# max-andr/joint-cnn-mrf

Measured on AMD Instinct MI355X. Metric: images/sec (720x480, K=9 joints) part-detector+spatial-model fwd, higher is better.
Workload: dtype f32(fp16x2 spectra, fft); 1 GPU; configs[1]: batch=64/GPU synthetic 480x720x3, part detector + spatial model forward + argmax, fp32; batch_per_gpu=64, global_batch=64, micro_batch=64, use_sm=True, collective=all_gather coords int32 [B,2,9]

## Files before the change

include/jcm.h:

```cpp
#ifndef JCM_H
#define JCM_H

#include <stddef.h>
#include <stdint.h>

#ifdef __cplusplus
extern "C" {
#endif

typedef struct jcm_ctx* jcm_handle;

#define JCM_OK 0
#define JCM_ERR_ARG 1
#define JCM_ERR_STATE 2
#define JCM_ERR_HIP 3

#define JCM_PRECISION_F32 0
#define JCM_PRECISION_BF16 1

int jcm_create(int device, void* stream, jcm_handle* out);
int jcm_destroy(jcm_handle h);
const char* jcm_last_error(void);
int jcm_abi_version(void);

// ... 54 lines not shown
                    int32_t* disp, int64_t* sad);

int jcm_seq_tracks_viterbi(jcm_handle h, const float* hm, int S, int T, int HH, int WW, int M, const double* taps, int R, double rho, int D,
                           int32_t* path, double* maxes, int32_t* breaks, float* value);
int jcm_seq_tracks_filter(jcm_handle h, const float* hm, int S, int T, int HH, int WW, int M, const double* taps, int R, double rho, int D,
                          const double* state_in, float* filtered, int32_t* coords, double* norm, int32_t* reset, double* state_out, float* value);

int jcm_torso_infer(jcm_handle h, const float* prob, int B, int HH, int WW, int K, const int32_t* cells_in,
                    float* energy, int32_t* cell, float* torso);

int jcm_forward(jcm_handle h, const float* x, const float* torso, int B, int H, int W, int use_sm,
                float* pd_prob, float* sm_prob, int32_t* pd_coords, int32_t* sm_coords);

int jcm_eval_forward(jcm_handle h, const float* x, const float* y, int B, int H, int W, int use_sm,
                     float* pd_prob, float* sm_prob, int32_t* pd_coords, int32_t* sm_coords, float* losses);

int jcm_pd_forward_u8(jcm_handle h, const uint8_t* x, int B, int H, int W, float* logits_out);
int jcm_forward_u8(jcm_handle h, const uint8_t* x, const float* torso, int B, int H, int W, int use_sm,
                   float* pd_prob, float* sm_prob, int32_t* pd_coords, int32_t* sm_coords);
int jcm_eval_forward_u8(jcm_handle h, const uint8_t* x, const float* y, int B, int H, int W, int use_sm,
                        float* pd_prob, float* sm_prob, int32_t* pd_coords, int32_t* sm_coords, float* losses);

int jcm_window_resize(jcm_handle h, const float* src, int nsrc, int H, int W, int C, const int32_t* windows, int NW,
                      int OH, int OW, float* out);
int jcm_group_mean(jcm_handle h, const float* in, int n, int G, int64_t M, float* out);

int jcm_fit_images(jcm_handle h, const uint8_t* src, int64_t src_bytes, const int64_t* desc, int B, int C,
                   int OH, int OW, int pad, int out_f32, void* out, int32_t* geom);

int jcm_fit_windows(jcm_handle h, const uint8_t* src, int64_t src_bytes, const int64_t* desc, int NW, int C,
// ... 94 lines not shown
```

joint-cnn-mrf_amd/_lib.py:

```python
import ctypes
import os

_HERE = os.path.dirname(os.path.abspath(__file__))
LIB_PATH = os.environ.get('JCM_LIB') or os.path.join(_HERE, 'libjcm.so')

JCM_PRECISION_F32 = 0
JCM_PRECISION_BF16 = 1
JCM_OPT_ADAM = 0
JCM_OPT_MOMENTUM = 1
JCM_HIST_BUCKETS = 1551
SYNTH_REC_INTS, SYNTH_PRIM_INTS = 20, 16
HM_FLIP_PERM = (3, 4, 5, 0, 1, 2, 7, 6, 8, 9)

_c_float_p = ctypes.c_void_p
_c_i32_p = ctypes.c_void_p
_handle = ctypes.c_void_p
GRAD_READY_FN = ctypes.CFUNCTYPE(None, ctypes.c_void_p, ctypes.c_int64, ctypes.c_int64)

SIGNATURES = {
    'jcm_create': (ctypes.c_int, [ctypes.c_int, ctypes.c_void_p, ctypes.POINTER(_handle)]),
    'jcm_destroy': (ctypes.c_int, [_handle]),
    'jcm_last_error': (ctypes.c_char_p, []),
    'jcm_abi_version': (ctypes.c_int, []),
    'jcm_set_option': (ctypes.c_int, [_handle, ctypes.c_char_p, ctypes.c_int64]),
# ... 38 lines not shown
                                      ctypes.c_void_p]),
    'jcm_seq_smooth_lag': (ctypes.c_int, [_handle, _c_float_p, ctypes.c_int, ctypes.c_int, ctypes.c_int, ctypes.c_int, ctypes.c_int, ctypes.c_int,
                                          ctypes.POINTER(ctypes.c_double), ctypes.c_int, ctypes.c_double, ctypes.c_int, ctypes.c_int, ctypes.c_void_p,
                                          ctypes.c_void_p, _c_i32_p, _c_float_p, _c_i32_p, _c_float_p, ctypes.c_void_p, _c_i32_p]),
    'jcm_seq_tracks_viterbi': (ctypes.c_int, [_handle, _c_float_p, ctypes.c_int, ctypes.c_int, ctypes.c_int, ctypes.c_int, ctypes.c_int,
                                              ctypes.POINTER(ctypes.c_double), ctypes.c_int, ctypes.c_double, ctypes.c_int, _c_i32_p, ctypes.c_void_p, _c_i32_p,
                                              _c_float_p]),
    'jcm_seq_tracks_filter': (ctypes.c_int, [_handle, _c_float_p, ctypes.c_int, ctypes.c_int, ctypes.c_int, ctypes.c_int, ctypes.c_int,
                                             ctypes.POINTER(ctypes.c_double), ctypes.c_int, ctypes.c_double, ctypes.c_int, ctypes.c_void_p, _c_float_p, _c_i32_p,
                                             ctypes.c_void_p, _c_i32_p, ctypes.c_void_p, _c_float_p]),
    'jcm_frame_shift': (ctypes.c_int, [_handle, ctypes.c_void_p, ctypes.c_int, ctypes.c_int, ctypes.c_int, ctypes.c_int, ctypes.c_int, ctypes.c_int, ctypes.c_int,
                                       ctypes.c_int, ctypes.c_void_p, _c_i32_p, ctypes.c_void_p]),
    'jcm_torso_infer': (ctypes.c_int, [_handle, _c_float_p, ctypes.c_int, ctypes.c_int, ctypes.c_int, ctypes.c_int, _c_i32_p, _c_float_p, _c_i32_p, _c_float_p]),
    'jcm_forward': (ctypes.c_int, [_handle, _c_float_p, _c_float_p, ctypes.c_int, ctypes.c_int, ctypes.c_int, ctypes.c_int,
                                   _c_float_p, _c_float_p, _c_i32_p, _c_i32_p]),
    'jcm_eval_forward': (ctypes.c_int, [_handle, _c_float_p, _c_float_p, ctypes.c_int, ctypes.c_int, ctypes.c_int, ctypes.c_int,
                                        _c_float_p, _c_float_p, _c_i32_p, _c_i32_p, _c_float_p]),
    'jcm_pd_forward_u8': (ctypes.c_int, [_handle, ctypes.c_void_p, ctypes.c_int, ctypes.c_int, ctypes.c_int, _c_float_p]),
    'jcm_forward_u8': (ctypes.c_int, [_handle, ctypes.c_void_p, _c_float_p, ctypes.c_int, ctypes.c_int, ctypes.c_int, ctypes.c_int,
                                      _c_float_p, _c_float_p, _c_i32_p, _c_i32_p]),
    'jcm_eval_forward_u8': (ctypes.c_int, [_handle, ctypes.c_void_p, _c_float_p, ctypes.c_int, ctypes.c_int, ctypes.c_int, ctypes.c_int,
                                           _c_float_p, _c_float_p, _c_i32_p, _c_i32_p, _c_float_p]),
    'jcm_window_resize': (ctypes.c_int, [_handle, _c_float_p, ctypes.c_int, ctypes.c_int, ctypes.c_int, ctypes.c_int,
                                         ctypes.POINTER(ctypes.c_int32), ctypes.c_int, ctypes.c_int, ctypes.c_int, _c_float_p]),
    'jcm_fit_images': (ctypes.c_int, [_handle, ctypes.c_void_p, ctypes.c_int64, ctypes.POINTER(ctypes.c_int64), ctypes.c_int, ctypes.c_int, ctypes.c_int,
                                      ctypes.c_int, ctypes.c_int, ctypes.c_int, ctypes.c_void_p, ctypes.POINTER(ctypes.c_int32)]),
    'jcm_fit_windows': (ctypes.c_int, [_handle, ctypes.c_void_p, ctypes.c_int64, ctypes.POINTER(ctypes.c_int64), ctypes.c_int, ctypes.c_int, ctypes.c_int,
                                       ctypes.c_int, ctypes.c_int, ctypes.c_int, ctypes.c_void_p, ctypes.POINTER(ctypes.c_int32)]),
    'jcm_render_poses': (ctypes.c_int, [_handle, ctypes.c_void_p, ctypes.c_int64, ctypes.POINTER(ctypes.c_int64), ctypes.c_int, ctypes.c_void_p,
                                        ctypes.POINTER(ctypes.c_int32), ctypes.c_int, _c_float_p, ctypes.c_int, ctypes.c_int, ctypes.c_int, ctypes.c_int,
# ... 113 lines not shown
```

joint-cnn-mrf_amd/csrc/ctx.h:

```cpp
#pragma once
#include "../../include/jcm.h"

#include <map>
#include <mutex>
#include <string>
#include <vector>

#include "kernels.h"

namespace jcm {

struct CallOrder;

int fail(int code, const std::string& msg);

#define HIP_TRY(expr)                                                                                   \
  do {                                                                                                  \
    hipError_t e_ = (expr);                                                                             \
    if (e_ != hipSuccess)                                                                               \
      return ::jcm::fail(JCM_ERR_HIP, std::string(#expr) + ": " + hipGetErrorString(e_));               \
  } while (0)
#define JCM_TRY(expr)          \
  do {                         \
    int r_ = (expr);           \
// ... 51 lines not shown
  int device = 0;
  hipStream_t stream = nullptr;
  int precision = JCM_PRECISION_F32;
  int K = 9;
  bool finalized = false;
  int f32_conv = 0;
  int split_min_wgs = 128;
  int sm_algo = 3;
  int conv9_fft = 1;
  int fft_tiles = 1;
  int fft_logits_rows = 1;
  int fft_fuse = 7;
  int fft_single = 1;
  int fft_t16 = 1;
  int fft_rows_mfma = 1;
  int fft_reg = 1;
  int fft_cache_gb = 64;
  int fft_win = 1;
  int bf16_hpool = 1;
  int torso_algo = 1;
  int sm_chunk = 32;
  int micro_batch = 0;
  int call_order = 1;
  int debug_skip = 0;
  std::map<std::string, jcm::Tensor> params;
  std::map<std::string, jcm::ConvLayer> convs;
  std::vector<void*> owned;
  size_t param_bytes = 0;
  bool has_sm = false;
  float* sp_energy = nullptr;
// ... 150 lines not shown
template <class F>
int with_arena(jcm_ctx* c, F&& body) {
  return with_arena(c, body, body);
}

bool conv1_pool_fused(const jcm_ctx* c, const ConvLayer* L1, int H, int W);
bool conv1_split_route(const jcm_ctx* c, const ConvLayer* L1);
int conv1_pool_stage(jcm_ctx* c, const std::string& scope, const ConvLayer* L1, const void* xin, bool xin_u8, int B, int xh, int xw, int xsub, void* dst, void** p1);
struct Pool2Layout {
  int pl23;
  int hp;
};
Pool2Layout pool2_layout(jcm_ctx* c, const ConvLayer* L2, const ConvLayer* L3, int B, int h2, int w2);
hipError_t pool2_launch(jcm_ctx* c, const Pool2Layout& l, const void* c2, void* p2, int B, int h2, int w2, int C);
int pd_forward_impl(jcm_ctx* c, const void* x, bool x_u8, int B, int H, int W, float* logits);
int sm_forward_impl(jcm_ctx* c, const float* hm, int Ca, const float* extra, int B, float* logits, int extra_ld = 0);

}
```

joint-cnn-mrf_amd/csrc/jcm_api.hip:

```cpp
#include <algorithm>
#include <cmath>
#include <cstdlib>
#include <cstdio>
#include <cstring>

#include <mutex>
#include <vector>

#include "ctx.h"
#include "options.h"

using namespace jcm;

namespace {
thread_local std::string g_err;
}

namespace jcm {

const char* const kJointNames[10] = {"lsho", "lelb", "lwri", "rsho", "relb", "rwri", "lhip", "rhip", "nose", "torso"};

int fail(int code, const std::string& msg) {
  g_err = msg;
  return code;
// ... 594 lines not shown
  CallOrder order(h);
  HIP_TRY(softmax_argmax(logits, prob, coords, B, HH * WW, WW, K, h->stream));
  return JCM_OK;
}

int jcm_argmax_coords(jcm_handle h, const float* hm, int B, int HH, int WW, int K, int32_t* coords) {
  JCM_TRY(check(h, false));
  if (!hm || !coords || B < 1 || HH < 1 || WW < 1 || K < 1) return fail(JCM_ERR_ARG, "bad argmax arguments");
  DeviceGuard g(h->device);
  CallOrder order(h);
  HIP_TRY(argmax_coords(hm, coords, B, HH * WW, WW, K, h->stream));
  return JCM_OK;
}

static int forward_impl(jcm_handle h, const void* x, bool x_u8, const float* torso, const float* y, int B, int H, int W, int use_sm,
                        float* pd_prob, float* sm_prob, int32_t* pd_coords, int32_t* sm_coords, float* losses) {
  JCM_TRY(check(h, true));
  if (!x || B < 1 || H < 8 || W < 8) return fail(JCM_ERR_ARG, "bad forward arguments");
  const int tld = y ? h->K + 1 : 1;
  if (y) torso = y + h->K;
  if (use_sm && !torso) return fail(JCM_ERR_ARG, "use_sm needs the torso heat map (y_in[...,K:], main.py:528)");
  if (use_sm && (cdiv2(cdiv2(cdiv2(H))) != kHmH || cdiv2(cdiv2(cdiv2(W))) != kHmW))
    return fail(JCM_ERR_ARG, "the spatial model is defined for 60x90 heat maps (480x720 images) only");
  DeviceGuard g(h->device);
  CallOrder order(h);
  jcm_ctx* c = h;
  const int K = c->K;
  if (use_sm && K + 1 != kC) return fail(JCM_ERR_ARG, "use_sm requires n_joints == 9 (10-channel spatial model)");
  const int hh = cdiv2(cdiv2(cdiv2(H))), ww = cdiv2(cdiv2(cdiv2(W)));
  const int mb_opt = c->micro_batch > 0 ? c->micro_batch : (c->precision == JCM_PRECISION_BF16 ? 256 : 64);
  const int mb = B < mb_opt ? B : mb_opt;
  auto body = [&](int b0, int nb) {
    const size_t n = (size_t)nb * hh * ww * K;
    const size_t o = (size_t)b0 * hh * ww * K;
    float* logits = arena_alloc<float>(c, n);
    float* prob = pd_prob ? pd_prob + o : arena_alloc<float>(c, n);
    const size_t mark = c->arena_off;
    const void* xb = static_cast<const char*>(x) + (size_t)b0 * H * W * 3 * (x_u8 ? 1 : sizeof(float));
    JCM_TRY(pd_forward_impl(c, xb, x_u8, nb, H, W, logits));
    c->arena_off = mark;
    if (!c->dry) HIP_TRY(softmax_argmax(logits, prob, pd_coords ? pd_coords + (size_t)b0 * 2 * K : nullptr, nb, hh * ww, ww, K, c->stream));
    float* ce = losses ? arena_alloc<float>(c, 2 * (size_t)nb * K) : nullptr;
    const float* yb = y ? y + (size_t)b0 * hh * ww * (K + 1) : nullptr;
    if (losses && !c->dry) HIP_TRY(softmax_ce(logits, yb, nb, hh * ww, K, K + 1, 0.f, ce, nullptr, 0, 0, c->stream));
    if (use_sm) {
      float* sml = arena_alloc<float>(c, n);
      float* smp = sm_prob ? sm_prob + o : nullptr;
      hipEvent_t s0 = nullptr, s1 = nullptr;
      if (!c->dry) JCM_TRY(prof_begin(c, &s0, &s1));
      const int rs = sm_forward_impl(c, prob, K, torso + (size_t)b0 * hh * ww * tld, nb, sml, tld);
      if (!c->dry) prof_end(c, "sm", s0, s1, rs == JCM_OK);
      JCM_TRY(rs);
      if (!c->dry && (smp || sm_coords))
        HIP_TRY(softmax_argmax(sml, smp, sm_coords ? sm_coords + (size_t)b0 * 2 * K : nullptr, nb, hh * ww, ww, K, c->stream));
      if (losses && !c->dry) HIP_TRY(softmax_ce(sml, yb, nb, hh * ww, K, K + 1, 0.f, ce + (size_t)nb * K, nullptr, 0, 0, c->stream));
    } else if (losses && !c->dry) {
      HIP_TRY(hipMemcpyAsync(ce + (size_t)nb * K, ce, (size_t)nb * K * sizeof(float), hipMemcpyDeviceToDevice, c->stream));
    }
    if (losses && !c->dry) HIP_TRY(loss_means_accumulate(ce, nb * K, 1.0f / (float)(B * K), losses, b0 == 0, c->stream));
    return (int)JCM_OK;
  };
  return with_arena(c, [&] { return body(0, mb); }, [&] {
    for (int b0 = 0; b0 < B; b0 += mb) {
      c->arena_off = 0;
      JCM_TRY(body(b0, B - b0 < mb ? B - b0 : mb));
    }
    return (int)JCM_OK;
  });
}

int jcm_forward(jcm_handle h, const float* x, const float* torso, int B, int H, int W, int use_sm,
                float* pd_prob, float* sm_prob, int32_t* pd_coords, int32_t* sm_coords) {
  return forward_impl(h, x, false, torso, nullptr, B, H, W, use_sm, pd_prob, sm_prob, pd_coords, sm_coords, nullptr);
}
int jcm_forward_u8(jcm_handle h, const uint8_t* x, const float* torso, int B, int H, int W, int use_sm,
                   float* pd_prob, float* sm_prob, int32_t* pd_coords, int32_t* sm_coords) {
  return forward_impl(h, x, true, torso, nullptr, B, H, W, use_sm, pd_prob, sm_prob, pd_coords, sm_coords, nullptr);
}

int jcm_eval_forward(jcm_handle h, const float* x, const float* y, int B, int H, int W, int use_sm,
                     float* pd_prob, float* sm_prob, int32_t* pd_coords, int32_t* sm_coords, float* losses) {
  if (!y || !losses) return fail(JCM_ERR_ARG, "eval_forward needs the target heat maps y [B,60,90,K+1] and a 2-float loss buffer");
  return forward_impl(h, x, false, nullptr, y, B, H, W, use_sm, pd_prob, sm_prob, pd_coords, sm_coords, losses);
}
int jcm_eval_forward_u8(jcm_handle h, const uint8_t* x, const float* y, int B, int H, int W, int use_sm,
                        float* pd_prob, float* sm_prob, int32_t* pd_coords, int32_t* sm_coords, float* losses) {
  if (!y || !losses) return fail(JCM_ERR_ARG, "eval_forward needs the target heat maps y [B,60,90,K+1] and a 2-float loss buffer");
  return forward_impl(h, x, true, nullptr, y, B, H, W, use_sm, pd_prob, sm_prob, pd_coords, sm_coords, losses);
// ... 390 lines not shown
```

joint-cnn-mrf_amd/csrc/kernels.h:

```cpp
#pragma once
#include <hip/hip_runtime.h>
#include <stdint.h>

#include <atomic>

namespace jcm {

struct LdsAttr {
  std::atomic<uint64_t> done{0};
  hipError_t ensure(const void* fn, int bytes) {
    int dev = 0;
    hipError_t e = hipGetDevice(&dev);
    if (e != hipSuccess) return e;
    const uint64_t bit = 1ull << (dev & 63);
    if (done.load(std::memory_order_acquire) & bit) return hipSuccess;
    e = hipFuncSetAttribute(fn, hipFuncAttributeMaxDynamicSharedMemorySize, bytes);
    if (e == hipSuccess) done.fetch_or(bit, std::memory_order_release);
    return e;
  }
};

struct ConvArgs {
  const void* x;
  const void* wp;
// ... 259 lines not shown

hipError_t sm_softplus5(const float* in, float* out, int64_t n, hipStream_t st);
hipError_t sm_softplus5_multi(const float* const* in, float* out, int P, int64_t n, hipStream_t st);
hipError_t sm_likelihood(const float* hm, int Ca, const float* extra, const float* bn_scale, const float* bn_shift, float* lik,
                         int B, int C, hipStream_t st, int extra_ld = 0);
hipError_t sm_pair_conv(const float* priors, const float* maps, const int* cond, float* cpre,
                        int B, int P, int C, hipStream_t st);
hipError_t sm_finish(const float* lik, const float* cpre, const float* spbias, float* logits,
                     int B, int K, int C, hipStream_t st);
hipError_t sm_resize_only(const float* cpre, float* out, int B, hipStream_t st);

hipError_t sm_pad_frame(const float* hm, int Ca, const float* extra, const float* sc, const float* sh, float* frame, int B, int C,
                        hipStream_t st, int extra_ld = 0);
hipError_t sm_spec_mul(const float2* lhat, const float2* phat, const int* cond, float2* spec, int B, int C, int P, hipStream_t st);
hipError_t sm_resize_frame(const float* cfull, float* out, int B, hipStream_t st);
hipError_t sm_fused_forward(const float* hm, int Ca, const float* extra, int extra_ld, const float* sc, const float* sh, const float2* phat_t,
                            const int* cond, const float* spbias, float2* lhat_t, float* logits, int B, int K, int C, hipStream_t st,
                            float* tsave, void* scratch, unsigned epoch);
size_t sm_fused_scratch_bytes();
hipError_t sm_fused_spectra(const float* hm, int Ca, const float* extra, int extra_ld, const float* sc, const float* sh, float2* lhat_t, int B, int C,
                            hipStream_t st);
hipError_t sm_lds_fwd_frames(const float* frames, float2* spec_t, int n, hipStream_t st);
hipError_t sm_lds_fwd_dframes(const float* G, const float* T, float2* dhat_t, int nb, int K, int P, hipStream_t st);
hipError_t sm_lds_inv_frames(const float2* spec_t, float* frames, int n, int r0, int nrows, float scale, hipStream_t st);

hipError_t window_resize(const float* src, int H, int W, int C, const int* windows_dev, int NW, float2* mm_scratch,
                         int OH, int OW, float* out, hipStream_t st);
hipError_t group_mean(const float* in, float* out, int n, int G, size_t M, hipStream_t st);

size_t augment_scratch_doubles(int B);
hipError_t augment_train(const float* x, const float* y, const float* params, int B, int H, int W, int hh, int hw, double* scratch,
                         float* x_out, float* y_out, hipStream_t st);

// ... 79 lines not shown
```

joint-cnn-mrf_amd/csrc/options.h:

```cpp
#pragma once
#include <climits>

#include "ctx.h"

namespace jcm {

struct Option {
  enum Kind { BOOL, RANGE, EITHER };
  const char* name;
  int jcm_ctx::*field;
  Kind kind;
  int64_t lo, hi;
  bool before_finalize;
  const char* env;
  int (*on_change)(jcm_ctx*, int64_t);
};

int option_profile(jcm_ctx* c, int64_t value);
int option_fft_single(jcm_ctx* c, int64_t value);

inline constexpr Option kOptions[] = {
    {"precision",       &jcm_ctx::precision,       Option::RANGE,  0,  1,       true,  nullptr,               nullptr},
    {"n_joints",        &jcm_ctx::K,               Option::RANGE,  1,  9,       true,  nullptr,               nullptr},
    {"f32_conv",        &jcm_ctx::f32_conv,        Option::EITHER, 0,  2,       true,  nullptr,               nullptr},
    {"split_min_wgs",   &jcm_ctx::split_min_wgs,   Option::RANGE,  0,  INT_MAX, false, nullptr,               nullptr},
    {"profile",         &jcm_ctx::profile,         Option::BOOL,   0,  1,       false, nullptr,               option_profile},
    {"conv9_fft",       &jcm_ctx::conv9_fft,       Option::BOOL,   0,  1,       false, nullptr,               nullptr},
    {"call_order",      &jcm_ctx::call_order,      Option::BOOL,   0,  1,       false, nullptr,               nullptr},
    {"fft_single",      &jcm_ctx::fft_single,      Option::BOOL,   0,  1,       false, nullptr,               option_fft_single},
    {"fft_t16",         &jcm_ctx::fft_t16,         Option::BOOL,   0,  1,       false, nullptr,               nullptr},
    {"fft_rows_mfma",   &jcm_ctx::fft_rows_mfma,   Option::BOOL,   0,  1,       false, nullptr,               nullptr},
    {"fft_windows",     &jcm_ctx::fft_win,         Option::BOOL,   0,  1,       false, nullptr,               nullptr},
    {"fft_fuse",        &jcm_ctx::fft_fuse,        Option::RANGE,  0,  7,       false, nullptr,               nullptr},
    {"fft_tiles",       &jcm_ctx::fft_tiles,       Option::BOOL,   0,  1,       false, "JCM_FFT_TILES",       nullptr},
    {"fft_logits_rows", &jcm_ctx::fft_logits_rows, Option::BOOL,   0,  1,       false, "JCM_FFT_LOGITS_ROWS", nullptr},
    {"fft_reg",         &jcm_ctx::fft_reg,         Option::BOOL,   0,  1,       false, "JCM_FFT_REG",         nullptr},
    {"fft_cache_gb",    &jcm_ctx::fft_cache_gb,    Option::RANGE,  0,  1 << 20, false, "JCM_FFT_CACHE_GB",    nullptr},
    {"bf16_hpool",      &jcm_ctx::bf16_hpool,      Option::BOOL,   0,  1,       false, nullptr,               nullptr},
    {"sm_algo",         &jcm_ctx::sm_algo,         Option::EITHER, 1,  3,       false, nullptr,               nullptr},
    {"torso_algo",      &jcm_ctx::torso_algo,      Option::EITHER, 1,  1,       false, nullptr,               nullptr},
    {"sm_chunk",        &jcm_ctx::sm_chunk,        Option::RANGE,  1,  INT_MAX, false, nullptr,               nullptr},
    {"micro_batch",     &jcm_ctx::micro_batch,     Option::RANGE,  0,  INT_MAX, false, nullptr,               nullptr},
    {"debug_skip",      &jcm_ctx::debug_skip,      Option::RANGE,  0,  127,     false, nullptr,               nullptr},
};

}
```

joint-cnn-mrf_amd/csrc/pd_tower.hip:

```cpp
#include <string>
#include <utility>

#include "ctx.h"

namespace jcm {

bool conv1_pool_fused(const jcm_ctx* c, const ConvLayer* L1, int H, int W) {
  return (c->precision == JCM_PRECISION_BF16 ? L1->wq1_bf16 != nullptr : L1->wq1_f32 != nullptr) && H % 4 == 0 && W % 4 == 0;
}
bool conv1_split_route(const jcm_ctx* c, const ConvLayer* L1) { return c->conv9_fft && c->f32_conv == 0 && L1->wq1_split; }

int conv1_pool_stage(jcm_ctx* c, const std::string& scope, const ConvLayer* L1, const void* xin, bool xin_u8, int B, int xh, int xw, int xsub, void* dst, void** p1) {
  const bool bf = c->precision == JCM_PRECISION_BF16;
  const size_t es = bf ? 2 : 4;
  auto act = [&](size_t elems) { return static_cast<void*>(arena_alloc<char>(c, elems * es)); };
  const int h1 = cdiv2(xh / xsub), w1 = cdiv2(xw / xsub);
  const int h2 = cdiv2(h1), w2 = cdiv2(w1);
  if (conv1_pool_fused(c, L1, xh / xsub, xw / xsub)) {
    *p1 = dst ? dst : act((size_t)B * h2 * w2 * L1->cout);
    if (c->dry) return JCM_OK;
    if (bf) {
      HIP_TRY(conv1_mfma_pool(xin, L1->wq1_bf16, L1->bias, L1->scale, L1->shift, *p1, B, xh, xw, xsub, c->stream, xin_u8));
    } else {
      HIP_TRY(conv1_split_route(c, L1) ? conv1_mfma_pool_split(xin, L1->wq1_split, L1->bias, L1->scale, L1->shift, static_cast<float*>(*p1), B, xh, xw, xsub, c->stream, xin_u8)
// ... 204 lines not shown
  }
  const int sk = c->debug_skip;
  void* t56 = (sk & 96) ? nullptr : offer_handover(c, L5, conv_of(c, "conv6"), B, hh, ww, k5);
  void* c5 = t56 ? nullptr : act((size_t)B * hh * ww * L5->cout);
  if (fuse_merge) k5.merge = &mg;
  ConvCall q5 = conv_call(merged, c5, B, hh, ww);
  q5.act_bf16 = bf; q5.in_planar = planar45; q5.out_planar = planar; q5.link = &k5;
  if (!(sk & 32)) JCM_TRY(run_conv(c, "conv5", q5));
  hand_over(k5, k6);
  ConvCall q6 = conv_call(c5, logits, B, hh, ww);
  q6.act_bf16 = bf; q6.out_f32 = true; q6.in_planar = planar; q6.link = &k6;
  if (!(sk & 64)) JCM_TRY(run_conv(c, "conv6", q6));
  return JCM_OK;
}

int sm_forward_impl(jcm_ctx* c, const float* hm, int Ca, const float* extra, int B, float* logits, int extra_ld) {
  if (extra_ld <= 0) extra_ld = kC - Ca;
  if (!c->has_sm) return fail(JCM_ERR_STATE, "spatial-model parameters (bn_sm, energy_*, bias_*) were not set");
  const int P = c->K * (kC - 1);
  if (c->sm_algo == 1) {
    float* lik = arena_alloc<float>(c, (size_t)B * kC * kHmH * 96);
    float* cpre = arena_alloc<float>(c, (size_t)B * P * kCH * kCW);
    if (c->dry) return JCM_OK;
    HIP_TRY(sm_likelihood(hm, Ca, extra, c->bn_sm_scale, c->bn_sm_shift, lik, B, kC, c->stream, extra_ld));
    HIP_TRY(sm_pair_conv(c->sp_energy, lik, c->cond, cpre, B, P, kC, c->stream));
    HIP_TRY(sm_finish(lik, cpre, c->sp_bias, logits, B, c->K, kC, c->stream));
    return JCM_OK;
  }
  if (c->sm_algo == 3) {
    float2* lhat_t = arena_alloc<float2>(c, (size_t)B * kC * kSpec);
    if (c->dry) return JCM_OK;
    void* scr = nullptr;
    unsigned epoch = 0;
    JCM_TRY(sm_scratch_next(c, &scr, &epoch));
    HIP_TRY(sm_fused_forward(hm, Ca, extra, extra_ld, c->bn_sm_scale, c->bn_sm_shift, c->prior_spec_t, c->cond, c->sp_bias, lhat_t, logits, B, c->K, kC,
                             c->stream, nullptr, scr, epoch));
    return JCM_OK;
  }
  return fail(JCM_ERR_STATE, "sm_algo must be 3 (transforms in LDS) or 1 (direct)");
}

}
```

joint-cnn-mrf_amd/csrc/sm_fused.hip:

```cpp
#include <atomic>

#include "sm_lds_fft.h"

namespace jcm {


using namespace smf;

__global__ __launch_bounds__(NT) void sm_fwd_spectra_kernel(const float* __restrict__ hm, int Ca, const float* __restrict__ extra, int extra_ld,
                                                              const float* __restrict__ sc, const float* __restrict__ sh, float2* __restrict__ lhat_t, int C) {
  extern __shared__ __attribute__((aligned(16))) char smem[];
  cf* lds = reinterpret_cast<cf*>(smem);
  cf* cb = lds + CB;
  cf* rb = lds + RB;
  const int tid = threadIdx.x;
  const int b = blockIdx.x / C, c = blockIdx.x - b * C;
  make_twiddles(lds, tid);
  for (int i = tid; i < NROWP * PX; i += NT) rb[i] = cf{0.f, 0.f};
  for (int i = tid; i < WC * PU; i += NT) cb[i] = cf{0.f, 0.f};
  __syncthreads();
  float* rbf = reinterpret_cast<float*>(rb);
  for (int pix = tid; pix < MHW; pix += NT) {
    const int y = pix / MW, x = pix - y * MW;
    rbf[((y >> 1) * PX + x) * 2 + (y & 1)] = lik_of(hm, Ca, extra, extra_ld, sc, sh, (int64_t)b * MHW + pix, c);
// ... 3 lines not shown
  for (int t = tid; t < (MH / 2) * WC; t += NT) {
    const int i = t / WC, k = t - i * WC;
    const cf zk = rb[i * PX + pos180(k)], zn = rb[i * PX + pos180(k == 0 ? 0 : FW - k)];
    cb[k * PU + 2 * i] = cf{0.5f * (zk.x + zn.x), 0.5f * (zk.y - zn.y)};
    cb[k * PU + 2 * i + 1] = cf{0.5f * (zk.y + zn.y), -0.5f * (zk.x - zn.x)};
  }
  __syncthreads();
  fft120<PU, -1, WC>(cb, lds + TW120, tid);
  cf* __restrict__ out = reinterpret_cast<cf*>(lhat_t) + (size_t)blockIdx.x * (WC * FH);
  for (int e = tid; e < WC * FH; e += NT) {
    const int v = e / FH, u = e - v * FH;
    out[e] = cb[v * PU + pos120(u)];
  }
}

__global__ __launch_bounds__(NT) void sm_inv_finish_kernel(const float* __restrict__ hm, int Ca, const float* __restrict__ extra, int extra_ld,
                                                             const float* __restrict__ sc, const float* __restrict__ sh,
                                                             const float2* __restrict__ lhat_t, const float2* __restrict__ phat_t,
                                                             const int* __restrict__ cond, const float* __restrict__ spb, float* __restrict__ logits, int K,
                                                             int C, float* __restrict__ tsave, int nunits, float* __restrict__ part, unsigned* __restrict__ flags,
                                                             unsigned epoch, bool per_item) {
  extern __shared__ __attribute__((aligned(16))) char smem[];
  cf* lds = reinterpret_cast<cf*>(smem);
  cf* cb = lds + CB;
  cf* rb = lds + RB;
  const int tid = threadIdx.x;
  const int PJ = C - 1;
  make_twiddles(lds, tid);
  for (int t = tid; t < MH + MW; t += NT) {
    const bool isy = t < MH;
    const int o = isy ? t : t - MH;
    const float f = __fmul_rn((float)o, isy ? 61.0f / 60.0f : 91.0f / 90.0f);
    const int lo = (int)floorf(f), hi = min(lo + 1, isy ? 60 : 90);
    const int olo = isy ? ((lo >> 1) * PX) * 2 + (lo & 1) : 2 * pos180(89 + lo);
    const int ohi = isy ? ((hi >> 1) * PX) * 2 + (hi & 1) : 2 * pos180(89 + hi);
    lds[TY + t] = cf{__uint_as_float((unsigned)olo | ((unsigned)ohi << 16)), f - (float)lo};
// ... 112 lines not shown
      }
    }
    __syncthreads();
    if (seg_last) {
      if (in_head) {
        float* __restrict__ ps = part + (size_t)w * MHW;
#pragma unroll
        for (int i = 0; i < NPIX; ++i) {
          const int pix = tix + i * NT;
          if (pix < MHW) __builtin_nontemporal_store(e[i], ps + pix);
        }
        __builtin_amdgcn_fence(__ATOMIC_RELEASE, "agent");
        __syncthreads();
        if (tid == 0) __hip_atomic_store(flags + w, epoch, __ATOMIC_RELEASE, __HIP_MEMORY_SCOPE_AGENT);
      } else {
#pragma unroll
        for (int i = 0; i < NPIX; ++i) {
          const int pix = tix + i * NT;
          if (pix < MHW) logits[((size_t)b * MHW + pix) * K + j] = e[i];
        }
      }
    }
  }
}

static int sm_inv_resident() {
  static std::atomic<int> cached[64];
  int dev = 0;
  (void)hipGetDevice(&dev);
  int r = cached[dev & 63].load(std::memory_order_relaxed);
  if (r > 0) return r;
  int ncu = 256, per_cu = 0;
  (void)hipDeviceGetAttribute(&ncu, hipDeviceAttributeMultiprocessorCount, dev);
  if (hipOccupancyMaxActiveBlocksPerMultiprocessor(&per_cu, sm_inv_finish_kernel, NT, (size_t)LDS_BYTES) != hipSuccess || per_cu < 1) per_cu = 1;
  r = ncu * per_cu;
  cached[dev & 63].store(r, std::memory_order_relaxed);
  return r;
}
size_t sm_fused_scratch_bytes() { return (size_t)sm_inv_resident() * (MHW * sizeof(float) + 64); }

hipError_t sm_fused_forward(const float* hm, int Ca, const float* extra, int extra_ld, const float* sc, const float* sh, const float2* phat_t,
                            const int* cond, const float* spbias, float2* lhat_t, float* logits, int B, int K, int C, hipStream_t st, float* tsave, void* scratch,
                            unsigned epoch) {
  if (extra_ld <= 0) extra_ld = C - Ca;
  if (!scratch || epoch == 0) return hipErrorInvalidValue;
  static LdsAttr attr_f, attr_i;
  if (hipError_t e = attr_f.ensure(reinterpret_cast<const void*>(sm_fwd_spectra_kernel), LDS_BYTES); e != hipSuccess) return e;
  if (hipError_t e = attr_i.ensure(reinterpret_cast<const void*>(sm_inv_finish_kernel), LDS_BYTES); e != hipSuccess) return e;
  hipLaunchKernelGGL(sm_fwd_spectra_kernel, dim3(B * C), dim3(NT), LDS_BYTES, st, hm, Ca, extra, extra_ld, sc, sh, lhat_t, C);
  if (hipError_t e = hipGetLastError(); e != hipSuccess) return e;
  const int resident = sm_inv_resident();
  const int items = B * K, rounds = (items + resident - 1) / resident;
  int G = items;
  if (items > resident && (double)rounds * resident > 1.15 * (double)items) G = resident;
  if (G != items && (G % 8 != 0 || items / 8 < G / 8)) G = items;
  const bool per_item = G == items;
  if (per_item) G = 8 * ((B + 7) / 8) * K;
  float* part = static_cast<float*>(scratch);
  unsigned* flags = reinterpret_cast<unsigned*>(static_cast<char*>(scratch) + (size_t)resident * MHW * sizeof(float));
  hipLaunchKernelGGL(sm_inv_finish_kernel, dim3(G), dim3(NT), LDS_BYTES, st, hm, Ca, extra, extra_ld, sc, sh, lhat_t, phat_t, cond, spbias, logits, K, C, tsave, B * K * (C - 1),
                     part, flags, epoch, per_item);
  return hipGetLastError();
}


hipError_t sm_fused_spectra(const float* hm, int Ca, const float* extra, int extra_ld, const float* sc, const float* sh, float2* lhat_t, int B, int C,
                            hipStream_t st) {
  if (extra_ld <= 0) extra_ld = C - Ca;
  static LdsAttr attr_f;
  if (hipError_t e = attr_f.ensure(reinterpret_cast<const void*>(sm_fwd_spectra_kernel), LDS_BYTES); e != hipSuccess) return e;
  hipLaunchKernelGGL(sm_fwd_spectra_kernel, dim3(B * C), dim3(NT), LDS_BYTES, st, hm, Ca, extra, extra_ld, sc, sh, lhat_t, C);
  return hipGetLastError();
}

}
```

joint-cnn-mrf_amd/engine.py:

```python
import ctypes

import numpy as np
import torch

from . import _lib, motion
from .motion import SEQ_EXCLUDE


def _hm_size(n):
    for _ in range(3):
        n = (n + 1) // 2
    return n


def _precision(name):
    return {'fp32': _lib.JCM_PRECISION_F32, 'f32': _lib.JCM_PRECISION_F32, 'bf16': _lib.JCM_PRECISION_BF16}[name]


def _f32_conv(name):
    if name not in ('exact', 'split16'):
        raise ValueError("f32_conv must be 'exact' or 'split16' (the bf16x6 arm 'split' was retired in round 5)")
    return {'exact': 0, 'split16': 2}[name]


# ... 595 lines not shown
    def _tower_call(self, entry, x, maps, use_sm, want_prob, peaks, decode, torso, losses=False):
        B, H, W, _ = x.shape
        hh, ww, K = _hm_size(H), _hm_size(W), self.n_joints
        r, scratch = {}, {}
        for key in ('pd', 'sm') if use_sm else ('pd',):
            r[key + '_coords'] = self._new(B, 2, K, dtype=torch.int32)
            if want_prob or peaks:
                (r if want_prob else scratch)[key + '_prob'] = self._new(B, hh, ww, K)
        if losses:
            r['losses'] = self._new(2)
        what = entry + ('_u8' if x.dtype == torch.uint8 else '')
        _lib.check(getattr(self._lib, what)(self._h, self._p(x), self._p(maps), B, H, W, int(bool(use_sm)),
                                            self._p(r.get('pd_prob', scratch.get('pd_prob'))), self._p(r.get('sm_prob', scratch.get('sm_prob'))),
                                            self._p(r['pd_coords']), self._p(r.get('sm_coords')), *([self._p(r['losses'])] if losses else [])), what)
        return self._add_peaks_pose(r, scratch, peaks, decode, torso)

    def _forward_flip(self, x, torso, use_sm, want_prob, peaks, decode):
        r2 = self.forward(self.mirror_pairs(x), self.mirror_pairs(torso) if use_sm else None, use_sm=use_sm, want_prob=True)
        r, scratch = {}, {}
        for key in (('pd', 'sm') if use_sm else ('pd',)):
            self._on_stream(r2[key + '_prob'])
            prob = self.mirror_merge(r2[key + '_prob'])
            r[key + '_coords'] = self.argmax_coords(prob)
            (r if want_prob else scratch)[key + '_prob'] = prob
        return self._add_peaks_pose(r, scratch, peaks, decode, torso)

    def eval_forward(self, x, y, use_sm=True, want_prob=True, peaks=0, decode=False):
        self._chk_decode(decode, use_sm, peaks)
        self._chk_img(x, 'x')
        self._chk(y, 4, 'y')
# ... 426 lines not shown
```

Before: 7902 images/sec.

## Fuse part-detector softmax/argmax and SM softmax-argmax into spatial-model FFT kernels

Folds the part-detector softmax+argmax into the first spatial-model FFT kernel, which now reads the logits directly, writes the probabilities and coordinates, and builds the spectrum in LDS. The spatial-model softmax-argmax is also fused into the inverse/finish kernel, so the SM logits need not be written when only coordinates are requested. This removes two separate softmax_argmax launches and a logits round trip through global memory. In exchange it adds per-block reductions and an exact-equality argmax trick (e>0.99999 && e/s==1/s) that could change tie-breaking. A forward_from_logits entry point is added as well.

```diff
diff --git a/include/jcm.h b/include/jcm.h
--- a/include/jcm.h
+++ b/include/jcm.h
@@ -92,6 +92,9 @@
 
 int jcm_eval_forward(jcm_handle h, const float* x, const float* y, int B, int H, int W, int use_sm,
                      float* pd_prob, float* sm_prob, int32_t* pd_coords, int32_t* sm_coords, float* losses);
+
+int jcm_forward_from_logits(jcm_handle h, const float* logits, const float* torso, int B, int HH, int WW, int use_sm,
+                            float* pd_prob, float* sm_prob, int32_t* pd_coords, int32_t* sm_coords);
 
 int jcm_pd_forward_u8(jcm_handle h, const uint8_t* x, int B, int H, int W, float* logits_out);
 int jcm_forward_u8(jcm_handle h, const uint8_t* x, const float* torso, int B, int H, int W, int use_sm,
diff --git a/joint-cnn-mrf_amd/_lib.py b/joint-cnn-mrf_amd/_lib.py
--- a/joint-cnn-mrf_amd/_lib.py
+++ b/joint-cnn-mrf_amd/_lib.py
@@ -76,6 +76,8 @@
     'jcm_torso_infer': (ctypes.c_int, [_handle, _c_float_p, ctypes.c_int, ctypes.c_int, ctypes.c_int, ctypes.c_int, _c_i32_p, _c_float_p, _c_i32_p, _c_float_p]),
     'jcm_forward': (ctypes.c_int, [_handle, _c_float_p, _c_float_p, ctypes.c_int, ctypes.c_int, ctypes.c_int, ctypes.c_int,
                                    _c_float_p, _c_float_p, _c_i32_p, _c_i32_p]),
+    'jcm_forward_from_logits': (ctypes.c_int, [_handle, _c_float_p, _c_float_p, ctypes.c_int, ctypes.c_int, ctypes.c_int, ctypes.c_int,
+                                               _c_float_p, _c_float_p, _c_i32_p, _c_i32_p]),
     'jcm_eval_forward': (ctypes.c_int, [_handle, _c_float_p, _c_float_p, ctypes.c_int, ctypes.c_int, ctypes.c_int, ctypes.c_int,
                                         _c_float_p, _c_float_p, _c_i32_p, _c_i32_p, _c_float_p]),
     'jcm_pd_forward_u8': (ctypes.c_int, [_handle, ctypes.c_void_p, ctypes.c_int, ctypes.c_int, ctypes.c_int, _c_float_p]),
diff --git a/joint-cnn-mrf_amd/csrc/ctx.h b/joint-cnn-mrf_amd/csrc/ctx.h
--- a/joint-cnn-mrf_amd/csrc/ctx.h
+++ b/joint-cnn-mrf_amd/csrc/ctx.h
@@ -89,6 +89,7 @@
   int fft_single = 1;
   int fft_t16 = 1;
   int fft_rows_mfma = 1;
+  int tail_fuse = 1;
   int fft_reg = 1;
   int fft_cache_gb = 64;
   int fft_win = 1;
@@ -269,6 +270,7 @@
 Pool2Layout pool2_layout(jcm_ctx* c, const ConvLayer* L2, const ConvLayer* L3, int B, int h2, int w2);
 hipError_t pool2_launch(jcm_ctx* c, const Pool2Layout& l, const void* c2, void* p2, int B, int h2, int w2, int C);
 int pd_forward_impl(jcm_ctx* c, const void* x, bool x_u8, int B, int H, int W, float* logits);
-int sm_forward_impl(jcm_ctx* c, const float* hm, int Ca, const float* extra, int B, float* logits, int extra_ld = 0);
-
-}
+int sm_forward_impl(jcm_ctx* c, const float* hm, int Ca, const float* extra, int B, float* logits, int extra_ld = 0, const SmTail* tail = nullptr);
+bool sm_tail_fusable(const jcm_ctx* c, int Ca);
+
+}
diff --git a/joint-cnn-mrf_amd/csrc/jcm_api.hip b/joint-cnn-mrf_amd/csrc/jcm_api.hip
--- a/joint-cnn-mrf_amd/csrc/jcm_api.hip
+++ b/joint-cnn-mrf_amd/csrc/jcm_api.hip
@@ -632,9 +632,9 @@
 }
 
 static int forward_impl(jcm_handle h, const void* x, bool x_u8, const float* torso, const float* y, int B, int H, int W, int use_sm,
-                        float* pd_prob, float* sm_prob, int32_t* pd_coords, int32_t* sm_coords, float* losses) {
+                        float* pd_prob, float* sm_prob, int32_t* pd_coords, int32_t* sm_coords, float* losses, const float* given_logits = nullptr) {
   JCM_TRY(check(h, true));
-  if (!x || B < 1 || H < 8 || W < 8) return fail(JCM_ERR_ARG, "bad forward arguments");
+  if ((!x && !given_logits) || B < 1 || H < 8 || W < 8) return fail(JCM_ERR_ARG, "bad forward arguments");
   const int tld = y ? h->K + 1 : 1;
   if (y) torso = y + h->K;
   if (use_sm && !torso) return fail(JCM_ERR_ARG, "use_sm needs the torso heat map (y_in[...,K:], main.py:528)");
@@ -651,13 +651,18 @@
   auto body = [&](int b0, int nb) {
     const size_t n = (size_t)nb * hh * ww * K;
     const size_t o = (size_t)b0 * hh * ww * K;
-    float* logits = arena_alloc<float>(c, n);
+    float* own_logits = arena_alloc<float>(c, n);
+    const float* logits = given_logits ? given_logits + o : own_logits;
     float* prob = pd_prob ? pd_prob + o : arena_alloc<float>(c, n);
-    const size_t mark = c->arena_off;
-    const void* xb = static_cast<const char*>(x) + (size_t)b0 * H * W * 3 * (x_u8 ? 1 : sizeof(float));
-    JCM_TRY(pd_forward_impl(c, xb, x_u8, nb, H, W, logits));
-    c->arena_off = mark;
-    if (!c->dry) HIP_TRY(softmax_argmax(logits, prob, pd_coords ? pd_coords + (size_t)b0 * 2 * K : nullptr, nb, hh * ww, ww, K, c->stream));
+    if (!given_logits) {
+      const size_t mark = c->arena_off;
+      const void* xb = static_cast<const char*>(x) + (size_t)b0 * H * W * 3 * (x_u8 ? 1 : sizeof(float));
+      JCM_TRY(pd_forward_impl(c, xb, x_u8, nb, H, W, own_logits));
+      c->arena_off = mark;
+    }
+    const bool fuse = use_sm && sm_tail_fusable(c, K);
+    int32_t* pdc = pd_coords ? pd_coords + (size_t)b0 * 2 * K : nullptr;
+    if (!c->dry && !fuse) HIP_TRY(softmax_argmax(logits, prob, pdc, nb, hh * ww, ww, K, c->stream));
     float* ce = losses ? arena_alloc<float>(c, 2 * (size_t)nb * K) : nullptr;
     const float* yb = y ? y + (size_t)b0 * hh * ww * (K + 1) : nullptr;
     if (losses && !c->dry) HIP_TRY(softmax_ce(logits, yb, nb, hh * ww, K, K + 1, 0.f, ce, nullptr, 0, 0, c->stream));
@@ -666,11 +671,13 @@
       float* smp = sm_prob ? sm_prob + o : nullptr;
       hipEvent_t s0 = nullptr, s1 = nullptr;
       if (!c->dry) JCM_TRY(prof_begin(c, &s0, &s1));
-      const int rs = sm_forward_impl(c, prob, K, torso + (size_t)b0 * hh * ww * tld, nb, sml, tld);
+      int32_t* smc = sm_coords ? sm_coords + (size_t)b0 * 2 * K : nullptr;
+      const bool smc_fused = fuse && smc && !smp;
+      const SmTail tail{logits, prob, pdc, smc_fused ? smc : nullptr};
+      const int rs = sm_forward_impl(c, prob, K, torso + (size_t)b0 * hh * ww * tld, nb, smc_fused && !losses ? nullptr : sml, tld, fuse ? &tail : nullptr);
       if (!c->dry) prof_end(c, "sm", s0, s1, rs == JCM_OK);
       JCM_TRY(rs);
-      if (!c->dry && (smp || sm_coords))
-        HIP_TRY(softmax_argmax(sml, smp, sm_coords ? sm_coords + (size_t)b0 * 2 * K : nullptr, nb, hh * ww, ww, K, c->stream));
+      if (!c->dry && (smp || smc) && !smc_fused) HIP_TRY(softmax_argmax(sml, smp, smc, nb, hh * ww, ww, K, c->stream));
       if (losses && !c->dry) HIP_TRY(softmax_ce(sml, yb, nb, hh * ww, K, K + 1, 0.f, ce + (size_t)nb * K, nullptr, 0, 0, c->stream));
     } else if (losses && !c->dry) {
       HIP_TRY(hipMemcpyAsync(ce + (size_t)nb * K, ce, (size_t)nb * K * sizeof(float), hipMemcpyDeviceToDevice, c->stream));
@@ -690,6 +697,11 @@
 int jcm_forward(jcm_handle h, const float* x, const float* torso, int B, int H, int W, int use_sm,
                 float* pd_prob, float* sm_prob, int32_t* pd_coords, int32_t* sm_coords) {
   return forward_impl(h, x, false, torso, nullptr, B, H, W, use_sm, pd_prob, sm_prob, pd_coords, sm_coords, nullptr);
+}
+int jcm_forward_from_logits(jcm_handle h, const float* logits, const float* torso, int B, int HH, int WW, int use_sm,
+                            float* pd_prob, float* sm_prob, int32_t* pd_coords, int32_t* sm_coords) {
+  if (!logits || HH < 1 || WW < 1) return fail(JCM_ERR_ARG, "bad forward_from_logits arguments");
+  return forward_impl(h, nullptr, false, torso, nullptr, B, 8 * HH, 8 * WW, use_sm, pd_prob, sm_prob, pd_coords, sm_coords, nullptr, logits);
 }
 int jcm_forward_u8(jcm_handle h, const uint8_t* x, const float* torso, int B, int H, int W, int use_sm,
                    float* pd_prob, float* sm_prob, int32_t* pd_coords, int32_t* sm_coords) {
diff --git a/joint-cnn-mrf_amd/csrc/kernels.h b/joint-cnn-mrf_amd/csrc/kernels.h
--- a/joint-cnn-mrf_amd/csrc/kernels.h
+++ b/joint-cnn-mrf_amd/csrc/kernels.h
@@ -297,9 +297,15 @@
                         hipStream_t st, int extra_ld = 0);
 hipError_t sm_spec_mul(const float2* lhat, const float2* phat, const int* cond, float2* spec, int B, int C, int P, hipStream_t st);
 hipError_t sm_resize_frame(const float* cfull, float* out, int B, hipStream_t st);
+struct SmTail {
+  const float* pd_logits;
+  float* prob;
+  int32_t* pd_coords;
+  int32_t* sm_coords;
+};
 hipError_t sm_fused_forward(const float* hm, int Ca, const float* extra, int extra_ld, const float* sc, const float* sh, const float2* phat_t,
                             const int* cond, const float* spbias, float2* lhat_t, float* logits, int B, int K, int C, hipStream_t st,
-                            float* tsave, void* scratch, unsigned epoch);
+                            float* tsave, void* scratch, unsigned epoch, const SmTail* tail = nullptr);
 size_t sm_fused_scratch_bytes();
 hipError_t sm_fused_spectra(const float* hm, int Ca, const float* extra, int extra_ld, const float* sc, const float* sh, float2* lhat_t, int B, int C,
                             hipStream_t st);
diff --git a/joint-cnn-mrf_amd/csrc/options.h b/joint-cnn-mrf_amd/csrc/options.h
--- a/joint-cnn-mrf_amd/csrc/options.h
+++ b/joint-cnn-mrf_amd/csrc/options.h
@@ -35,6 +35,7 @@
     {"fft_tiles",       &jcm_ctx::fft_tiles,       Option::BOOL,   0,  1,       false, "JCM_FFT_TILES",       nullptr},
     {"fft_logits_rows", &jcm_ctx::fft_logits_rows, Option::BOOL,   0,  1,       false, "JCM_FFT_LOGITS_ROWS", nullptr},
     {"fft_reg",         &jcm_ctx::fft_reg,         Option::BOOL,   0,  1,       false, "JCM_FFT_REG",         nullptr},
+    {"tail_fuse",       &jcm_ctx::tail_fuse,       Option::BOOL,   0,  1,       false, "JCM_TAIL_FUSE",       nullptr},
     {"fft_cache_gb",    &jcm_ctx::fft_cache_gb,    Option::RANGE,  0,  1 << 20, false, "JCM_FFT_CACHE_GB",    nullptr},
     {"bf16_hpool",      &jcm_ctx::bf16_hpool,      Option::BOOL,   0,  1,       false, nullptr,               nullptr},
     {"sm_algo",         &jcm_ctx::sm_algo,         Option::EITHER, 1,  3,       false, nullptr,               nullptr},
diff --git a/joint-cnn-mrf_amd/csrc/pd_tower.hip b/joint-cnn-mrf_amd/csrc/pd_tower.hip
--- a/joint-cnn-mrf_amd/csrc/pd_tower.hip
+++ b/joint-cnn-mrf_amd/csrc/pd_tower.hip
@@ -242,9 +242,12 @@
   return JCM_OK;
 }
 
-int sm_forward_impl(jcm_ctx* c, const float* hm, int Ca, const float* extra, int B, float* logits, int extra_ld) {
+bool sm_tail_fusable(const jcm_ctx* c, int Ca) { return c->tail_fuse && c->has_sm && c->sm_algo == 3 && c->K == 9 && Ca == c->K; }
+
+int sm_forward_impl(jcm_ctx* c, const float* hm, int Ca, const float* extra, int B, float* logits, int extra_ld, const SmTail* tail) {
   if (extra_ld <= 0) extra_ld = kC - Ca;
   if (!c->has_sm) return fail(JCM_ERR_STATE, "spatial-model parameters (bn_sm, energy_*, bias_*) were not set");
+  if (tail && !sm_tail_fusable(c, Ca)) return fail(JCM_ERR_STATE, "sm_forward_impl: the fused tail exists on the fused route with 9 joints only");
   const int P = c->K * (kC - 1);
   if (c->sm_algo == 1) {
     float* lik = arena_alloc<float>(c, (size_t)B * kC * kHmH * 96);
@@ -262,7 +265,7 @@
     unsigned epoch = 0;
     JCM_TRY(sm_scratch_next(c, &scr, &epoch));
     HIP_TRY(sm_fused_forward(hm, Ca, extra, extra_ld, c->bn_sm_scale, c->bn_sm_shift, c->prior_spec_t, c->cond, c->sp_bias, lhat_t, logits, B, c->K, kC,
-                             c->stream, nullptr, scr, epoch));
+                             c->stream, nullptr, scr, epoch, tail));
     return JCM_OK;
   }
   return fail(JCM_ERR_STATE, "sm_algo must be 3 (transforms in LDS) or 1 (direct)");
diff --git a/joint-cnn-mrf_amd/csrc/sm_fused.hip b/joint-cnn-mrf_amd/csrc/sm_fused.hip
--- a/joint-cnn-mrf_amd/csrc/sm_fused.hip
+++ b/joint-cnn-mrf_amd/csrc/sm_fused.hip
@@ -1,6 +1,7 @@
 #include <atomic>
 
 #include "sm_lds_fft.h"
+#include "softmax_map.h"
 
 namespace jcm {
 
@@ -41,12 +42,70 @@
   }
 }
 
+__global__ __launch_bounds__(NT) void sm_fwd_from_logits_kernel(const float* __restrict__ z, float* __restrict__ prob, int32_t* __restrict__ pd_coords, int Ca,
+                                                                  const float* __restrict__ extra, int extra_ld, const float* __restrict__ sc,
+                                                                  const float* __restrict__ sh, float2* __restrict__ lhat_t, int C, int B) {
+  extern __shared__ __attribute__((aligned(16))) char smem[];
+  cf* lds = reinterpret_cast<cf*>(smem);
+  cf* cb = lds + CB;
+  cf* rb = lds + RB;
+  const int tid = threadIdx.x;
+  const int n = (int)blockIdx.x / 8, b = (int)blockIdx.x % 8 + 8 * (n / C), c = n % C;
+  if (b >= B) return;
+  make_twiddles(lds, tid);
+  for (int i = tid; i < NROWP * PX; i += NT) rb[i] = cf{0.f, 0.f};
+  for (int i = tid; i < WC * PU; i += NT) cb[i] = cf{0.f, 0.f};
+  float* rbf = reinterpret_cast<float*>(rb);
+  if (c < Ca) {
+    float* red = reinterpret_cast<float*>(lds + TY);
+    float v[smap::NV];
+    bool on[smap::QPT];
+#pragma unroll
+    for (int j = 0; j < smap::QPT; ++j) {
+      on[j] = smap::owns(tid, j, MHW);
+#pragma unroll
+      for (int pp = 0; pp < 4; ++pp)
+        v[4 * j + pp] = on[j] ? z[((int64_t)b * MHW + smap::pixel_of(tid, j, pp)) * Ca + c] : -INFINITY;
+    }
+    const float s = smap::exp_sum(v, on, red, tid);
+    smap::normalise_argmax(v, on, s, red, tid, pd_coords, b, c, Ca, MW);
+#pragma unroll
+    for (int i = 0; i < smap::NV; ++i)
+      if (on[i >> 2]) {
+        const int pix = smap::pixel_of(tid, i >> 2, i & 3), y = pix / MW, x = pix - y * MW;
+        prob[((int64_t)b * MHW + pix) * Ca + c] = v[i];
+        rbf[((y >> 1) * PX + x) * 2 + (y & 1)] = sc ? softplus5(v[i] * sc[c] + sh[c]) : v[i];
+      }
+  } else {
+    __syncthreads();
+    for (int pix = tid; pix < MHW; pix += NT) {
+      const int y = pix / MW, x = pix - y * MW;
+      rbf[((y >> 1) * PX + x) * 2 + (y & 1)] = lik_of(prob, Ca, extra, extra_ld, sc, sh, (int64_t)b * MHW + pix, c);
+    }
+  }
+  __syncthreads();
+  fft180<PX, -1, MH / 2>(rb, lds + TW180, tid);
+  for (int t = tid; t < (MH / 2) * WC; t += NT) {
+    const int i = t / WC, k = t - i * WC;
+    const cf zk = rb[i * PX + pos180(k)], zn = rb[i * PX + pos180(k == 0 ? 0 : FW - k)];
+    cb[k * PU + 2 * i] = cf{0.5f * (zk.x + zn.x), 0.5f * (zk.y - zn.y)};
+    cb[k * PU + 2 * i + 1] = cf{0.5f * (zk.y + zn.y), -0.5f * (zk.x - zn.x)};
+  }
+  __syncthreads();
+  fft120<PU, -1, WC>(cb, lds + TW120, tid);
+  cf* __restrict__ out = reinterpret_cast<cf*>(lhat_t) + ((size_t)b * C + c) * (WC * FH);
+  for (int e = tid; e < WC * FH; e += NT) {
+    const int v = e / FH, u = e - v * FH;
+    out[e] = cb[v * PU + pos120(u)];
+  }
+}
+
 __global__ __launch_bounds__(NT) void sm_inv_finish_kernel(const float* __restrict__ hm, int Ca, const float* __restrict__ extra, int extra_ld,
                                                              const float* __restrict__ sc, const float* __restrict__ sh,
                                                              const float2* __restrict__ lhat_t, const float2* __restrict__ phat_t,
                                                              const int* __restrict__ cond, const float* __restrict__ spb, float* __restrict__ logits, int K,
                                                              int C, float* __restrict__ tsave, int nunits, float* __restrict__ part, unsigned* __restrict__ flags,
-                                                             unsigned epoch, bool per_item) {
+                                                             unsigned epoch, bool per_item, int32_t* __restrict__ coords) {
   extern __shared__ __attribute__((aligned(16))) char smem[];
   cf* lds = reinterpret_cast<cf*>(smem);
   cf* cb = lds + CB;
@@ -189,10 +248,31 @@
         __syncthreads();
         if (tid == 0) __hip_atomic_store(flags + w, epoch, __ATOMIC_RELEASE, __HIP_MEMORY_SCOPE_AGENT);
       } else {
-#pragma unroll
-        for (int i = 0; i < NPIX; ++i) {
-          const int pix = tix + i * NT;
-          if (pix < MHW) logits[((size_t)b * MHW + pix) * K + j] = e[i];
+        if (logits) {
+#pragma unroll
+          for (int i = 0; i < NPIX; ++i) {
+            const int pix = tix + i * NT;
+            if (pix < MHW) logits[((size_t)b * MHW + pix) * K + j] = e[i];
+          }
+        }
+        if (coords) {
+          float* ef = reinterpret_cast<float*>(cb);
+#pragma unroll
+          for (int i = 0; i < NPIX; ++i) {
+            const int pix = tix + i * NT;
+            if (pix < MHW) ef[pix] = e[i];
+          }
+          __syncthreads();
+          float v[smap::NV];
+          bool on[smap::QPT];
+#pragma unroll
+          for (int jj = 0; jj < smap::QPT; ++jj) {
+            on[jj] = smap::owns(tix, jj, MHW);
+#pragma unroll
+            for (int pp = 0; pp < 4; ++pp) v[4 * jj + pp] = on[jj] ? ef[smap::pixel_of(tix, jj, pp)] : -INFINITY;
+          }
+          const float s = smap::exp_sum(v, on, ef + MHW, tid);
+          smap::argmax_of_exp(v, on, s, ef + MHW, tid, coords, b, j, K, MW);
         }
       }
     }
@@ -216,13 +296,21 @@
 
 hipError_t sm_fused_forward(const float* hm, int Ca, const float* extra, int extra_ld, const float* sc, const float* sh, const float2* phat_t,
                             const int* cond, const float* spbias, float2* lhat_t, float* logits, int B, int K, int C, hipStream_t st, float* tsave, void* scratch,
-                            unsigned epoch) {
+                            unsigned epoch, const SmTail* tail) {
   if (extra_ld <= 0) extra_ld = C - Ca;
   if (!scratch || epoch == 0) return hipErrorInvalidValue;
-  static LdsAttr attr_f, attr_i;
-  if (hipError_t e = attr_f.ensure(reinterpret_cast<const void*>(sm_fwd_spectra_kernel), LDS_BYTES); e != hipSuccess) return e;
+  if (tail && (K != 9 || Ca != K || !tail->pd_logits || tail->prob != hm || tsave)) return hipErrorInvalidValue;
+  if (!logits && !(tail && tail->sm_coords)) return hipErrorInvalidValue;
+  static LdsAttr attr_f, attr_l, attr_i;
   if (hipError_t e = attr_i.ensure(reinterpret_cast<const void*>(sm_inv_finish_kernel), LDS_BYTES); e != hipSuccess) return e;
-  hipLaunchKernelGGL(sm_fwd_spectra_kernel, dim3(B * C), dim3(NT), LDS_BYTES, st, hm, Ca, extra, extra_ld, sc, sh, lhat_t, C);
+  if (tail) {
+    if (hipError_t e = attr_l.ensure(reinterpret_cast<const void*>(sm_fwd_from_logits_kernel), LDS_BYTES); e != hipSuccess) return e;
+    hipLaunchKernelGGL(sm_fwd_from_logits_kernel, dim3(8 * ((B + 7) / 8) * C), dim3(NT), LDS_BYTES, st, tail->pd_logits, tail->prob, tail->pd_coords, Ca, extra, extra_ld,
+                       sc, sh, lhat_t, C, B);
+  } else {
+    if (hipError_t e = attr_f.ensure(reinterpret_cast<const void*>(sm_fwd_spectra_kernel), LDS_BYTES); e != hipSuccess) return e;
+    hipLaunchKernelGGL(sm_fwd_spectra_kernel, dim3(B * C), dim3(NT), LDS_BYTES, st, hm, Ca, extra, extra_ld, sc, sh, lhat_t, C);
+  }
   if (hipError_t e = hipGetLastError(); e != hipSuccess) return e;
   const int resident = sm_inv_resident();
   const int items = B * K, rounds = (items + resident - 1) / resident;
@@ -234,7 +322,7 @@
   float* part = static_cast<float*>(scratch);
   unsigned* flags = reinterpret_cast<unsigned*>(static_cast<char*>(scratch) + (size_t)resident * MHW * sizeof(float));
   hipLaunchKernelGGL(sm_inv_finish_kernel, dim3(G), dim3(NT), LDS_BYTES, st, hm, Ca, extra, extra_ld, sc, sh, lhat_t, phat_t, cond, spbias, logits, K, C, tsave, B * K * (C - 1),
-                     part, flags, epoch, per_item);
+                     part, flags, epoch, per_item, tail ? tail->sm_coords : nullptr);
   return hipGetLastError();
 }
 
diff --git a/joint-cnn-mrf_amd/csrc/softmax_map.h b/joint-cnn-mrf_amd/csrc/softmax_map.h
--- /dev/null
+++ b/joint-cnn-mrf_amd/csrc/softmax_map.h
@@ -0,0 +1,119 @@
+#pragma once
+#include <hip/hip_runtime.h>
+
+#include <cmath>
+#include <cstdint>
+
+namespace jcm {
+namespace smap {
+
+constexpr int VT = 704, VW = VT / 64, QPT = 2, NV = 4 * QPT;
+constexpr int RED = 2 * VW;
+
+__device__ __forceinline__ int pixel_of(int tid, int j, int pp) { return 4 * (tid + j * VT) + pp; }
+__device__ __forceinline__ bool owns(int tid, int j, int HW) { return tid < VT && tid + j * VT < (HW >> 2); }
+
+__device__ __forceinline__ float wave_max(float v) {
+#pragma unroll
+  for (int o = 32; o > 0; o >>= 1) v = fmaxf(v, __shfl_xor(v, o));
+  return v;
+}
+__device__ __forceinline__ float wave_sum(float v) {
+#pragma unroll
+  for (int o = 32; o > 0; o >>= 1) v += __shfl_xor(v, o);
+  return v;
+}
+
+__device__ __forceinline__ float exp_sum(float (&v)[NV], const bool (&on)[QPT], float* red, int tid) {
+  const int wv = tid >> 6;
+  float a = -INFINITY;
+#pragma unroll
+  for (int i = 0; i < NV; ++i) a = fmaxf(a, v[i]);
+  a = wave_max(a);
+  if ((tid & 63) == 0 && wv < VW) red[wv] = a;
+  __syncthreads();
+  float m = red[0];
+#pragma unroll
+  for (int w = 1; w < VW; ++w) m = fmaxf(m, red[w]);
+  __syncthreads();
+  a = 0.f;
+#pragma unroll
+  for (int i = 0; i < NV; ++i) {
+    const float e = on[i >> 2] ? expf(v[i] - m) : 0.f;
+    v[i] = e;
+    a += e;
+  }
+  a = wave_sum(a);
+  if ((tid & 63) == 0 && wv < VW) red[wv] = a;
+  __syncthreads();
+  float s = red[0];
+#pragma unroll
+  for (int w = 1; w < VW; ++w) s += red[w];
+  __syncthreads();
+  return s;
+}
+
+__device__ __forceinline__ void store_coords(int bi, int32_t* __restrict__ coords, int b, int k, int K, int WW) {
+  if (bi == 0x7fffffff) bi = 0;
+  const int row = bi / WW;
+  coords[((size_t)b * 2 + 0) * K + k] = row;
+  coords[((size_t)b * 2 + 1) * K + k] = bi - row * WW;
+}
+
+__device__ __forceinline__ void normalise_argmax(float (&v)[NV], const bool (&on)[QPT], float s, float* red, int tid, int32_t* __restrict__ coords, int b,
+                                                 int k, int K, int WW) {
+  const int wv = tid >> 6;
+  int* redi = reinterpret_cast<int*>(red + VW);
+  float bv = -INFINITY;
+  int bi = 0x7fffffff;
+#pragma unroll
+  for (int i = 0; i < NV; ++i) {
+    const float pv = v[i] / s;
+    v[i] = pv;
+    const int pix = pixel_of(tid, i >> 2, i & 3);
+    if (on[i >> 2] && (pv > bv || (pv == bv && pix < bi))) { bv = pv; bi = pix; }
+  }
+  if (!coords) return;
+#pragma unroll
+  for (int o = 32; o > 0; o >>= 1) {
+    const float ov = __shfl_xor(bv, o);
+    const int oi = __shfl_xor(bi, o);
+    if (ov > bv || (ov == bv && oi < bi)) { bv = ov; bi = oi; }
+  }
+  if ((tid & 63) == 0 && wv < VW) { red[wv] = bv; redi[wv] = bi; }
+  __syncthreads();
+  if (tid == 0) {
+    bv = red[0];
+    bi = redi[0];
+    for (int w = 1; w < VW; ++w)
+      if (red[w] > bv || (red[w] == bv && redi[w] < bi)) { bv = red[w]; bi = redi[w]; }
+    store_coords(bi, coords, b, k, K, WW);
+  }
+  __syncthreads();
+}
+
+__device__ __forceinline__ void argmax_of_exp(const float (&v)[NV], const bool (&on)[QPT], float s, float* red, int tid, int32_t* __restrict__ coords, int b,
+                                              int k, int K, int WW) {
+  const int wv = tid >> 6;
+  int* redi = reinterpret_cast<int*>(red + VW);
+  const float pmax = 1.0f / s;
+  int bi = 0x7fffffff;
+#pragma unroll
+  for (int i = 0; i < NV; ++i) {
+    const float e = v[i];
+    if (on[i >> 2] && e > 0.99999f && e / s == pmax) bi = min(bi, pixel_of(tid, i >> 2, i & 3));
+  }
+#pragma unroll
+  for (int o = 32; o > 0; o >>= 1) bi = min(bi, __shfl_xor(bi, o));
+  if ((tid & 63) == 0 && wv < VW) redi[wv] = bi;
+  __syncthreads();
+  if (tid == 0) {
+    bi = redi[0];
+    for (int w = 1; w < VW; ++w) bi = min(bi, redi[w]);
+    store_coords(bi, coords, b, k, K, WW);
+  }
+  __syncthreads();
+}
+
+}
+}
diff --git a/joint-cnn-mrf_amd/engine.py b/joint-cnn-mrf_amd/engine.py
--- a/joint-cnn-mrf_amd/engine.py
+++ b/joint-cnn-mrf_amd/engine.py
@@ -633,6 +633,24 @@
                                             self._p(r.get('pd_prob', scratch.get('pd_prob'))), self._p(r.get('sm_prob', scratch.get('sm_prob'))),
                                             self._p(r['pd_coords']), self._p(r.get('sm_coords')), *([self._p(r['losses'])] if losses else [])), what)
         return self._add_peaks_pose(r, scratch, peaks, decode, torso)
+
+    def forward_from_logits(self, logits, torso=None, use_sm=True, want_prob=True):
+        self._chk(logits, 4, 'logits')
+        B, hh, ww, K = logits.shape
+        if K != self.n_joints or (use_sm and (torso is None or tuple(torso.shape) != (B, hh, ww, 1))):
+            raise ValueError('logits must be [B,H,W,%d] and, with use_sm, torso [B,H,W,1]; got %s, %s'
+                             % (self.n_joints, tuple(logits.shape), None if torso is None else tuple(torso.shape)))
+        if use_sm:
+            self._chk(torso, 4, 'torso')
+        r = {}
+        for key in ('pd', 'sm') if use_sm else ('pd',):
+            r[key + '_coords'] = self._new(B, 2, K, dtype=torch.int32)
+            if want_prob:
+                r[key + '_prob'] = self._new(B, hh, ww, K)
+        _lib.check(self._lib.jcm_forward_from_logits(self._h, self._p(logits), self._p(torso if use_sm else None), B, hh, ww, int(bool(use_sm)),
+                                                     self._p(r.get('pd_prob')), self._p(r.get('sm_prob')), self._p(r['pd_coords']),
+                                                     self._p(r.get('sm_coords'))), 'jcm_forward_from_logits')
+        return r
 
     def _forward_flip(self, x, torso, use_sm, want_prob, peaks, decode):
         r2 = self.forward(self.mirror_pairs(x), self.mirror_pairs(torso) if use_sm else None, use_sm=use_sm, want_prob=True)
```

Result: no change. 7979 images/sec, median of 6 (+1.0%).
